# chensh236/ComputerVisionImageStich2

Measured on AMD Instinct MI355X. Metric: warp+blend MPix/s at 4096x4096x3 f32, higher is better.
Workload: dtype f32 (f64 accumulators)

## Files before the change

computervisionimagestich2_amd/csrc/k_sweeps.inc:

```
constexpr int TS = 64;
constexpr int TP = 68;

__device__ __forceinline__ void tile_load(const float* __restrict__ base, int pitch, int c0, int lane, f4 pre[16]) {
    const float* p = base + (size_t)(lane >> 4) * pitch + c0 + ((lane & 15) << 2);
#pragma unroll
    for (int i = 0; i < 16; ++i) pre[i] = *reinterpret_cast<const f4*>(p + (size_t)(4 * i) * pitch);
}
__device__ __forceinline__ void tile_to_lds(float* tile, int lane, const f4 pre[16]) {
    float* t = tile + (lane >> 4) * TP + ((lane & 15) << 2);
#pragma unroll
    for (int i = 0; i < 16; ++i) *reinterpret_cast<f4*>(t + (4 * i) * TP) = pre[i];
}
__device__ __forceinline__ void tile_store(float* __restrict__ base, int pitch, int c0, int lane, const float* tile) {
    float* p = base + (size_t)(lane >> 4) * pitch + c0 + ((lane & 15) << 2);
    const float* t = tile + (lane >> 4) * TP + ((lane & 15) << 2);
#pragma unroll
    for (int i = 0; i < 16; ++i)
        __builtin_nontemporal_store(*reinterpret_cast<const f4*>(t + (4 * i) * TP), reinterpret_cast<f4*>(p + (size_t)(4 * i) * pitch));
}

struct Bands {
    int nr, h;
};

struct MaskL0 {
    const SeamDev* seam;
    float* side;
    int h;
    int enabled;
};
__device__ __forceinline__ float mask_step(const SeamDev& sd, int x) {
    return sd.branch == 0 ? ((double)x < sd.thr ? 1.f : 0.f) : (x >= sd.start ? 1.f : 0.f);
}

__device__ __forceinline__ void tile_store_rows(float* __restrict__ base, int pitch, int c0, int lane, const float* tile, int nrows) {
    float* p = base + (size_t)(lane >> 4) * pitch + c0 + ((lane & 15) << 2);
    const float* t = tile + (lane >> 4) * TP + ((lane & 15) << 2);
#pragma unroll
    for (int i = 0; i < 16; ++i)
        if ((lane >> 4) + 4 * i < nrows)
            __builtin_nontemporal_store(*reinterpret_cast<const f4*>(t + (4 * i) * TP), reinterpret_cast<f4*>(p + (size_t)(4 * i) * pitch));
}

template <typename PX>
__device__ __forceinline__ void mosaic_indices(const XShift& ms, int c0, int lane, int y0, int w, f4 nidx[16]) {
    const int c = c0 + ((lane & 15) << 2);
    const unsigned c0i = mosaic_col<PX>(ms, c, w), c1i = mosaic_col<PX>(ms, c + 1, w), c2i = mosaic_col<PX>(ms, c + 2, w),
                   c3i = mosaic_col<PX>(ms, c + 3, w);
#pragma unroll
    for (int i = 0; i < 16; ++i) {
        const unsigned row = mosaic_row<PX>(ms, y0 + (lane >> 4) + 4 * i);
        f4 v;
        v.x = __uint_as_float(mosaic_offset<PX>(row, c0i));
        v.y = __uint_as_float(mosaic_offset<PX>(row, c1i));
        v.z = __uint_as_float(mosaic_offset<PX>(row, c2i));
        v.w = __uint_as_float(mosaic_offset<PX>(row, c3i));
        nidx[i] = v;
    }
}
template <typename PX>
__device__ __forceinline__ float src_px(__amdgpu_buffer_rsrc_t rs, bool warped, unsigned byte_off) {
    const float v = buf_px<PX>(rs, byte_off);
    return warped ? warped_px<PX>(v) : v;
}
template <typename PX>
__device__ __forceinline__ void src_gather(__amdgpu_buffer_rsrc_t rs, const f4 nidx[16], f4 pre[16]) {
#pragma unroll
    for (int i = 0; i < 16; ++i) {
        const f4 id = nidx[i];
        f4 v;
        v.x = buf_raw<PX>(rs, __float_as_uint(id.x));
        v.y = buf_raw<PX>(rs, __float_as_uint(id.y));
        v.z = buf_raw<PX>(rs, __float_as_uint(id.z));
        v.w = buf_raw<PX>(rs, __float_as_uint(id.w));
        pre[i] = v;
    }
}
template <typename PX>
__device__ __forceinline__ void src_finish(bool warped, f4 pre[16]) {
#pragma unroll
    for (int i = 0; i < 16; ++i) {
        f4 v = pre[i];
#pragma unroll
        for (int j = 0; j < 4; ++j) {
            const float t = raw_to_px<PX>(v[j]);
            v[j] = warped ? warped_px<PX>(t) : t;
        }
        pre[i] = v;
    }
}

template <typename PX, bool SRC, bool CKPT = false>
__global__ __launch_bounds__(64) void k_vv_x_fwd(const float* __restrict__ in, float* __restrict__ out, int w, int pitch,
                                                  long lines, VVK k, double* __restrict__ state, MaskL0 mk,
                                                  typename CollapseSrc<PX, SRC>::type pa, ZeroTiles zt, ZeroTiles zi,
                                                  double* __restrict__ ckpt, Bands bd) {
    __shared__ __attribute__((aligned(16))) float tile[TS * TP];
    const int lane = threadIdx.x;
    long blk = blockIdx.x;
    if (SRC && bd.nr > 0 && bd.nr % 8 == 0) {
        const long nr = bd.nr, per_pair = 7 * nr, pr_ = blk / per_pair, r = blk % per_pair;
        const long band = (r / 56) * 8 + r % 8, q = (r / 8) % 7;
        blk = pr_ * per_pair + q * nr + band;
    }
    const long plane = bd.nr > 0 ? blk / bd.nr : 0;
    const int band_y0 = bd.nr > 0 ? (int)(blk % bd.nr) * TS : 0;
    const int nrows = bd.nr > 0 ? min(TS, bd.h - band_y0) : TS;
    const long line0 = bd.nr > 0 ? plane * bd.h + band_y0 : blk * TS, line = line0 + lane;
    const float* ib = in + (size_t)line0 * pitch;
    float* ob = out + (size_t)line0 * pitch;
    const int ntiles = (w + TS - 1) / TS;
    const bool live = lane < nrows && line < lines;
    bool gen_mask = false;
    SeamDev sd;
    int src_q = 0, src_y0 = 0, src_pr = 0;
    if (mk.enabled) {
        if (plane % 7 == 6) {
            if (band_y0 >= TS) return;
            gen_mask = true;
            sd = mk.seam[plane / 7];
        }
        src_q = (int)(plane % 7);
        src_pr = (int)(plane / 7);
        src_y0 = band_y0;
    }
    const bool gen_frame = SRC && !gen_mask && src_q < 3 && !a_is_dense(pa), gen_mosaic = SRC && !gen_mask && !gen_frame;
    const __amdgpu_buffer_rsrc_t rs = x_rsrc<PX>(pa, src_pr, src_q);
    const XShift ms = x_shift<PX>(pa, src_pr, src_q);
    const float* idx_rows = in + ((size_t)src_pr * 7 * bd.h + src_y0) * pitch;
    f4 nidx[SRC ? 16 : 1];
    auto tile_outside = [&](int t) -> bool {
        if constexpr (SRC) return gen_frame && zi.flags && zi.flags[zi.index(src_pr, src_y0 >> 6, t)];
        return false;
    };
    auto index_tile = [&](int t) {
        if constexpr (SRC)
            if (!tile_outside(t)) tile_load(idx_rows, pitch, t * TS, lane, nidx);
    };
    auto gen_tile = [&](int c0, f4 pre[16]) {
        f4 v;
        const int c = c0 + ((lane & 15) << 2);
        v.x = mask_step(sd, c);
        v.y = mask_step(sd, c + 1);
        v.z = mask_step(sd, c + 2);
        v.w = mask_step(sd, c + 3);
#pragma unroll
        for (int i = 0; i < 16; ++i) pre[i] = v;
    };
    double iplus = 0.0;
    if (live)
        iplus = gen_mask     ? (double)mask_step(sd, w - 1)
                : gen_frame  ? (double)src_px<PX>(rs, true, reinterpret_cast<const unsigned*>(idx_rows)[(size_t)lane * pitch + (w - 1)])
                : gen_mosaic ? (double)src_px<PX>(rs, false, mosaic_offset<PX>(mosaic_row<PX>(ms, src_y0 + lane), mosaic_col<PX>(ms, w - 1, w)))
                             : (double)in[(size_t)line * pitch + (w - 1)];
    double v1 = 0, v2 = 0, v3 = 0;
    f4 pre[16];
#define STITCH_X_FETCH(T)                                                      \
    do {                                                                       \
        if (gen_mask)                                                          \
            gen_tile((T) * TS, pre);                                           \
        else if constexpr (SRC) {                                              \
            if (tile_outside(T)) {                                             \
                _Pragma("unroll") for (int i_ = 0; i_ < 16; ++i_) pre[i_] = f4{0.f, 0.f, 0.f, 0.f}; \
            } else                                                             \
                src_gather<PX>(rs, nidx, pre);                                 \
            if ((T) + 1 < ntiles) {                                            \
                if (gen_frame)                                                 \
                    index_tile((T) + 1);                                       \
                else                                                           \
                    mosaic_indices<PX>(ms, ((T) + 1) * TS, lane, src_y0, w, nidx); \
            }                                                                  \
        } else                                                                 \
            tile_load(ib, pitch, (T) * TS, lane, pre);                         \
    } while (0)
    if constexpr (SRC) {
        if (gen_frame)
            index_tile(0);
        else if (gen_mosaic)
            mosaic_indices<PX>(ms, 0, lane, src_y0, w, nidx);
    }
    STITCH_X_FETCH(0);
    for (int t = 0; t < ntiles; ++t) {
        if (!CKPT && zt.flags && tile_outside(t) &&
            (t == 0 || __ballot(live && (__double_as_longlong(v1) | __double_as_longlong(v2) | __double_as_longlong(v3)) != 0) == 0)) {
            if (t + 1 < ntiles) STITCH_X_FETCH(t + 1);
            if (lane == 0) zt.flags[zt.index(plane, band_y0 / TS, t)] = 1;
            continue;
        }
        if constexpr (SRC)
            if (!gen_mask) src_finish<PX>(gen_frame, pre);
        tile_to_lds(tile, lane, pre);
        if (t + 1 < ntiles) STITCH_X_FETCH(t + 1);
        __syncthreads();
        float* row = tile + lane * TP;
        const int jmax = min(TS, w - t * TS);
        if (t == 0) v1 = v2 = v3 = (double)row[0] / k.sumsq;
        if (CKPT && t > 0 && live) {
            double* c = ckpt + (size_t)(3 * t) * lines + line;
            c[0] = v1;
            c[lines] = v2;
            c[2 * lines] = v3;
        }
        const int jfull = jmax & ~15;
        unsigned nz = 0;
        for (int jb = 0; jb < jfull; jb += 16) {
            float xs[16];
#pragma unroll
            for (int q = 0; q < 4; ++q) *reinterpret_cast<f4*>(xs + 4 * q) = *reinterpret_cast<const f4*>(row + jb + 4 * q);
#pragma unroll
            for (int u = 0; u < 16; ++u) {
                double v0 = (double)xs[u];
                v0 += v1 * k.f1;
                v0 += v2 * k.f2;
                v0 += v3 * k.f3;
                xs[u] = (float)v0;
                nz |= __float_as_uint(xs[u]);
                v3 = v2;
                v2 = v1;
                v1 = v0;
            }
            if (!CKPT) {
#pragma unroll
                for (int q = 0; q < 4; ++q) *reinterpret_cast<f4*>(row + jb + 4 * q) = *reinterpret_cast<const f4*>(xs + 4 * q);
            }
        }
        for (int j = jfull; j < jmax; ++j) {
            double v0 = (double)row[j];
            v0 += v1 * k.f1;
            v0 += v2 * k.f2;
            v0 += v3 * k.f3;
            const float f = (float)v0;
            if (!CKPT) row[j] = f;
            nz |= __float_as_uint(f);
            v3 = v2;
            v2 = v1;
            v1 = v0;
        }
        __syncthreads();
        if (zt.flags) {
            const bool zero = __ballot(live && nz != 0) == 0;
            if (lane == 0) zt.flags[zt.index(plane, band_y0 / TS, t)] = zero ? 1 : 0;
            if (zero) continue;
        }
        if (!CKPT) {
            if (nrows == TS)
                tile_store(ob, pitch, t * TS, lane, tile);
            else
                tile_store_rows(ob, pitch, t * TS, lane, tile, nrows);
        }
    }
    if (live) {
        state[line] = v1;
        state[lines + line] = v2;
        state[2 * lines + line] = v3;
        state[3 * lines + line] = iplus;
    }
}

#undef STITCH_X_FETCH

__device__ __forceinline__ void triggs(const VVK& k, double iplus, double& v1, double& v2, double& v3, float& first) {
    const double uplus = iplus / k.den, vplus = uplus / k.den, unp = v1 - uplus, unp1 = v2 - uplus, unp2 = v3 - uplus;
    const double n0 = (k.M[0] * unp + k.M[1] * unp1 + k.M[2] * unp2 + vplus) * k.sum;
    const double n1 = (k.M[3] * unp + k.M[4] * unp1 + k.M[5] * unp2 + vplus) * k.sum;
    const double n2 = (k.M[6] * unp + k.M[7] * unp1 + k.M[8] * unp2 + vplus) * k.sum;
    first = (float)n0;
    v3 = n2;
    v2 = n1;
    v1 = n0;
}

__global__ __launch_bounds__(64) void k_vv_x_bwd(float* __restrict__ data, int w, int pitch, long lines, VVK k,
                                                  const double* __restrict__ state, MaskL0 mk, Bands bd) {
    __shared__ __attribute__((aligned(16))) float tile[TS * TP];
    const int lane = threadIdx.x;
    const long blk = blockIdx.x, plane = bd.nr > 0 ? blk / bd.nr : 0;
    const int band_y0 = bd.nr > 0 ? (int)(blk % bd.nr) * TS : 0;
    const int nrows = bd.nr > 0 ? min(TS, bd.h - band_y0) : TS;
    const long line0 = bd.nr > 0 ? plane * bd.h + band_y0 : blk * TS, line = line0 + lane;
    float* side_row = nullptr;
    if (mk.enabled) {
        if (plane % 7 == 6) {
            if (band_y0 >= TS) return;
            side_row = mk.side + (size_t)(plane / 7) * pitch;
        }
    }
    float* base = data + (size_t)line0 * pitch;
    const int ntiles = (w + TS - 1) / TS;
    const bool live = lane < nrows && line < lines;
    double v1 = 0, v2 = 0, v3 = 0, iplus = 0;
    if (live) {
        v1 = state[line];
        v2 = state[lines + line];
        v3 = state[2 * lines + line];
        iplus = state[3 * lines + line];
    }
    float first;
    triggs(k, iplus, v1, v2, v3, first);
    f4 pre[16];
    tile_load(base, pitch, (ntiles - 1) * TS, lane, pre);
    for (int t = ntiles - 1; t >= 0; --t) {
        tile_to_lds(tile, lane, pre);
        if (t > 0) tile_load(base, pitch, (t - 1) * TS, lane, pre);
        __syncthreads();
        float* row = tile + lane * TP;
        int jtop = min(TS, w - t * TS);
        if (t == ntiles - 1) {
            row[jtop - 1] = first;
            --jtop;
        }
        const int jfull = jtop & ~15;
        if (jtop > jfull) {
            for (int j = jtop - 1; j >= jfull; --j) {
                double v0 = (double)row[j];
                v0 *= k.sum;
                v0 += v1 * k.f1;
                v0 += v2 * k.f2;
                v0 += v3 * k.f3;
                row[j] = (float)v0;
                v3 = v2;
                v2 = v1;
                v1 = v0;
            }
        }
        for (int jb = jfull - 16; jb >= 0; jb -= 16) {
            float xs[16];
#pragma unroll
            for (int q = 0; q < 4; ++q) *reinterpret_cast<f4*>(xs + 4 * q) = *reinterpret_cast<const f4*>(row + jb + 4 * q);
#pragma unroll
            for (int u = 15; u >= 0; --u) {
                double v0 = (double)xs[u];
                v0 *= k.sum;
                v0 += v1 * k.f1;
                v0 += v2 * k.f2;
                v0 += v3 * k.f3;
                xs[u] = (float)v0;
                v3 = v2;
                v2 = v1;
// ... 462 lines not shown
```

computervisionimagestich2_amd/csrc/stitch_band.inc:

```
namespace {
constexpr int BAND_HALO = 2;

struct BandLevel {
    int w = 0, h_full = 0, rows = 0, row0 = 0, pitch = 0;
    int halo = 0;
    size_t ps = 0;
    float* g = nullptr;
    float* e = nullptr;
    int32_t *ix = nullptr, *iy = nullptr;
    double *ax = nullptr, *ay = nullptr;
    int c4_xa = 0, c4_xb = 0, sh_eff = 0;
    float* origin_g() const { return g + (size_t)halo * pitch; }
    float* origin_e() const { return e + (size_t)halo * pitch; }
};
}

struct stitch_band {
    int device = 0, cw = 0, ch = 0, rank = 0, nranks = 1, Ls = 0, L = 0;
    stitch_blend_opts opts{};
    VVK vvk{};
    BandLevel lv[32];
    void* arena = nullptr;
    size_t arena_bytes = 0;
    float* T = nullptr;
// ... 59 lines not shown
        const int ph = a.rows + 2 * a.halo, ybase = a.row0 - a.halo;
        PairArgs<PX>& px = band_pa<PX>(b, false);
        PairArgs<PX>& pc = band_pa<PX>(b, true);
        px = pa, pc = pa;
        px.oy[0] = oy + ybase, pc.oy[0] = oy + a.row0;
        const ZeroTiles zi = band_zero_tiles(b, b->zi);
        if (zi.flags) k_fill_bytes<<<64, 256, 0, s>>>(zi.flags, (size_t)zi.NR * zi.NC, (uint8_t)1);
        k_src_index<PX><<<grid_xy(a.pitch, (ph + SI_ROWS - 1) / SI_ROWS, 1), 256, 0, s>>>(pa, a.g, a.w, ph, a.pitch, a.ps, zi, ybase);
        k_seam<PX><<<1, 256, 0, s>>>(nullptr, b->cw, b->ch, a.pitch, a.ps, b->opts.seam_rule, b->d_seam, pa, 1);
    } else {
        k_compose<PX><<<grid_xy(a.pitch, a.rows, 1), 256, 0, s>>>(pa, a.origin_g(), a.w, a.rows, a.pitch, a.ps, a.row0);
        k_seam<PX><<<1, 256, 0, s>>>(nullptr, b->cw, b->ch, a.pitch, a.ps, b->opts.seam_rule, b->d_seam, pa, 1);
        k_mask<<<grid_xy(a.pitch, a.rows, 1), 256, 0, s>>>(a.origin_g(), a.w, a.pitch, a.ps, b->d_seam);
    }
    HIPCHK(hipMemcpyAsync(b->h_seam, b->d_seam, sizeof(SeamDev), hipMemcpyDeviceToHost, s));
    b->last_stream = s, b->pending = true;
    return launch_check("band_compose");
}

template <typename OUT>
int band_collapse(stitch_band* b, int level, OUT* d_out, void* stream) {
    int rc = band_check(b, level, b->Ls - 1);
    if (rc) return rc;
    if (level == 0 && !d_out) return fail(STITCH_ERR_ARG, "band_collapse: level 0 needs the output band");
    hipStream_t s = as_stream(stream);
    const BandLevel& a = b->lv[level];
    const BandLevel& nx = b->lv[level + 1];
    const bool top_src = level + 1 == b->Ls;
    const float* gn = top_src ? b->gtop : nx.g;
    const float* en = top_src ? b->etop : nx.e;
    const int spitch = top_src ? nx.w : nx.pitch;
    const size_t sps = top_src ? (size_t)nx.w * nx.h_full : nx.ps;
    int xa = a.c4_xa, xb = a.c4_xb;
    const int crows = std::max(4, std::min(32, a.rows / 8));
    const int strips = (a.rows + crows - 1) / crows;
    if (level == 0) {
        if ((a.w % 4) != 0 || (reinterpret_cast<uintptr_t>(d_out) % (4 * sizeof(OUT))) != 0) xa = xb = 0;
        OutPtrs<OUT> outs{};
        outs.p[0] = d_out;
        if (b->src_l0 && b->px != (int)sizeof(OUT)) return fail(STITCH_ERR_ARG, "band_collapse: the output's pixel type differs from the composed inputs'");
        CollapseArgs<OUT, true> A{a.origin_g(), a.w, a.rows, a.pitch, a.ps, gn, en, nx.w, a.sh_eff, spitch, sps, {a.ix, a.ax, a.iy, a.ay}, outs,
                                  a.w, (size_t)a.w * a.rows, b->d_seam, b->src_l0 ? band_pa<OUT>(b, true) : PairArgs<OUT>{}, b->src_l0 ? 1 : 0, crows, xa, xb,
                                  1};
        const int rest = a.w - (xb - xa), nb4 = ((xb - xa) / 4 + WAVE - 1) / WAVE, ncb = (rest + C4_THREADS - 1) / C4_THREADS;
        if (xb > xa)
            k_collapse4<OUT, true><<<dim3(nb4 + ncb * C4_SUB, strips, 1), C4_THREADS, 0, s>>>(A, nb4, ncb);
        else
            k_collapse<OUT, true><<<grid_xy(a.w, strips, 1), 256, 0, s>>>(A);
    } else {
        OutPtrs<float> eo{};
        eo.p[0] = a.origin_e();
        CollapseArgs<float, false> A{a.origin_g(), a.w, a.rows, a.pitch, a.ps, gn, en, nx.w, a.sh_eff, spitch, sps, {a.ix, a.ax, a.iy, a.ay}, eo,
                                     a.pitch, a.ps, nullptr, NoPairArgs{}, 0, crows, xa, xb, 1};
        const int rest = a.pitch - (xb - xa), nb4 = ((xb - xa) / 4 + WAVE - 1) / WAVE, ncb = (rest + C4_THREADS - 1) / C4_THREADS;
        if (xb > xa)
            k_collapse4<float, false><<<dim3(nb4 + ncb * C4_SUB, strips, 1), C4_THREADS, 0, s>>>(A, nb4, ncb);
        else
            k_collapse<float, false><<<grid_xy(a.pitch, strips, 1), 256, 0, s>>>(A);
    }
    b->last_stream = s, b->pending = true;
    return launch_check("band_collapse");
}
}

namespace {
Bands band_bands(const stitch_band* b) {
    const int ph = b->lv[0].rows + 2 * b->lv[0].halo;
    return Bands{(ph + TS - 1) / TS, ph};
}
ZeroTiles band_zero_tiles(const stitch_band* b, uint8_t* flags, int level) {
    const BandLevel& a = b->lv[level];
    ZeroTiles z{};
    const int NR = (a.rows + TS - 1) / TS;
    if ((level > 0 || b->src_l0) && (a.w & 1) == 0 && NR <= 256 && a.halo == 0 && b->zero_tiles && !b->plain_dec) {
        z.flags = flags;
        z.h = a.rows;
        z.NR = NR;
        z.NC = (a.w + TS - 1) / TS;
    }
    return z;
}
int band_x_fwd_src(stitch_band* b, hipStream_t s, bool flags) {
    const BandLevel& a = b->lv[0];
    const Bands bd = band_bands(b);
    const long lines = 7L * bd.h;
    const ZeroTiles zt = flags ? band_zero_tiles(b, b->zt) : ZeroTiles{}, zi = band_zero_tiles(b, b->zi);
    if (b->px == 1)
        k_vv_x_fwd<uint8_t, true><<<7 * bd.nr, 64, 0, s>>>(a.g, b->T, a.w, a.pitch, lines, b->vvk, b->state_x, band_mask(b), b->pa8x, zt, zi, nullptr, bd);
    else if (b->px == 4)
        k_vv_x_fwd<float, true><<<7 * bd.nr, 64, 0, s>>>(a.g, b->T, a.w, a.pitch, lines, b->vvk, b->state_x, band_mask(b), b->pafx, zt, zi, nullptr, bd);
    else
        return fail(STITCH_ERR_ARG, "band: reduce before compose");
    return STITCH_OK;
}
}

extern "C" {

int stitch_band_create(int cw, int ch, int rank, int nranks, int split_levels, const stitch_blend_opts* opts, stitch_band** out) {
    if (!out) return fail(STITCH_ERR_ARG, "band_create: null output");
    *out = nullptr;
    int rc = need_device();
    if (rc) return rc;
    stitch_blend_opts o;
    stitch_blend_opts_default(&o);
    if (opts) o = *opts;
    if (o.blur_kind != 0 || o.level_rule != 0 || o.seam_rule != 0 || !(o.sigma >= 0.5f))
        return fail(STITCH_ERR_ARG, "band_create: the band split implements the root variant (Van Vliet blur, sigma >= 0.5)");
    if (nranks < 1 || rank < 0 || rank >= nranks) return fail(STITCH_ERR_ARG, "band_create: rank %d of %d", rank, nranks);
    int lw[32], lh[32];
    const int L = pyramid_levels(cw, ch, 0, lw, lh);
    if (L < 0) return L;
    const int Ls = split_levels;
    if (Ls < 1 || Ls > L - 1) return fail(STITCH_ERR_ARG, "band_create: split_levels must be 1..%d for a %d-level pyramid", L - 1, L);
    for (int l = 0; l <= Ls; ++l) {
        const int q = l < Ls ? 2 * nranks : nranks;
        if (lh[l] % q != 0 || lh[l] / nranks < (l < Ls ? 2 * BAND_HALO : 1))
            return fail(STITCH_ERR_ARG, "band_create: level %d has %d rows, not divisible into %d bands of even height >= %d", l, lh[l], nranks,
                        2 * BAND_HALO);
        if (lw[l] < 2) return fail(STITCH_ERR_ARG, "band_create: level %d is %d columns wide", l, lw[l]);
    }
    stitch_band* b = new stitch_band();
    b->cw = cw, b->ch = ch, b->rank = rank, b->nranks = nranks, b->Ls = Ls, b->L = L, b->opts = o;
    b->vvk = make_vvk(o.sigma);
    if (hipGetDevice(&b->device) != hipSuccess) {
        delete b;
        return fail(STITCH_ERR_HIP, "hipGetDevice failed");
    }
    size_t off = 0;
    auto take = [&](size_t bytes) {
        const size_t o2 = off;
        off += align256(bytes);
        return o2;
    };
    size_t g_off[32], e_off[32], ix_off[32], ax_off[32], iy_off[32], ay_off[32];
    for (int l = 0; l <= Ls; ++l) {
        BandLevel& v = b->lv[l];
        v.w = lw[l], v.h_full = lh[l], v.rows = lh[l] / nranks, v.row0 = rank * v.rows, v.pitch = round_up(v.w, 64);
        v.halo = l == 0 || nranks == 1 ? 0 : BAND_HALO;
        v.ps = (size_t)v.pitch * (v.rows + 2 * v.halo);
        g_off[l] = take(sizeof(float) * (v.ps * 7 + (size_t)v.pitch * 64));
        e_off[l] = (l >= 1 && l < Ls) ? take(sizeof(float) * v.ps * 3) : 0;
        if (l < Ls) {
            ix_off[l] = take(sizeof(int32_t) * v.w);
            ax_off[l] = take(sizeof(double) * v.w);
            iy_off[l] = take(sizeof(int32_t) * v.rows);
            ay_off[l] = take(sizeof(double) * v.rows);
        }
    }
    const BandLevel& v0 = b->lv[0];
    const size_t t_off = take(sizeof(float) * (v0.ps * 7 + (size_t)v0.pitch * 64));
    const size_t st_off = take(sizeof(double) * 4 * 7 * (size_t)(v0.rows + 2 * BAND_HALO + 64));
    const size_t seam_off = take(sizeof(SeamDev));
    const size_t side_off = take(sizeof(float) * v0.pitch);
    const size_t ntile0 = (size_t)((v0.rows + TS - 1) / TS) * ((v0.w + TS - 1) / TS);
    const size_t zt_off = take(7 * ntile0), zi_off = take(ntile0);
    const size_t yg_off = take(sizeof(u64) * (7 * (size_t)(v0.pitch / TS) * WF_GRAN * WAVE + 1));
    const size_t wfc_off = take(sizeof(unsigned) * 64);
    const size_t gtop_off = take(sizeof(float) * 7 * (size_t)lw[Ls] * lh[Ls]);
    const size_t etop_off = take(sizeof(float) * 3 * (size_t)lw[Ls] * lh[Ls]);
    b->arena_bytes = off;
    if (hipMalloc(&b->arena, off) != hipSuccess || hipMemset(b->arena, 0, off) != hipSuccess ||
        hipHostMalloc((void**)&b->h_seam, sizeof(SeamDev)) != hipSuccess || hipHostMalloc((void**)&b->h_wf_sticky, sizeof(unsigned)) != hipSuccess) {
        (void)hipGetLastError();
        stitch_band_destroy(b);
        return fail(STITCH_ERR_HIP, "band_create: allocation of %zu bytes failed", off);
    }
    std::memset(b->h_seam, 0, sizeof(SeamDev));
    *b->h_wf_sticky = 0;
    char* base = static_cast<char*>(b->arena);
    b->mask_side = reinterpret_cast<float*>(base + side_off);
    b->zt = reinterpret_cast<uint8_t*>(base + zt_off);
    b->zi = reinterpret_cast<uint8_t*>(base + zi_off);
// ... 318 lines not shown
```

computervisionimagestich2_amd/csrc/stitch_hip.hip:

```cpp
#include <hip/hip_runtime.h>

#include <cmath>
#include <cstdarg>
#include <cstdio>
#include <cstdlib>
#include <algorithm>
#include <cstring>
#include <atomic>
#include <condition_variable>
#include <functional>
#include <list>
#include <mutex>
#include <string>
#include <thread>
#include <vector>

#include "stitch.h"
#include "stitch_kernels.hpp"

#pragma clang fp contract(off)

using namespace sk;

namespace {
// ... 288 lines not shown

struct StageTimer {
    stitch_plan* p;
    hipStream_t s;
    ProfRec r{};
    bool on;
    StageTimer(stitch_plan* plan, hipStream_t st, int stage, int level)
        : p(plan), s(st), on(plan->profiling && (plan->prof_only < 0 || plan->prof_only == stage)) {
        if (!on) return;
        r.stage = stage;
        r.level = level;
        auto get = [&](hipEvent_t& e) {
            if (!p->free_events.empty()) {
                e = p->free_events.back();
                p->free_events.pop_back();
            } else
                (void)hipEventCreate(&e);
        };
        get(r.a);
        get(r.b);
        (void)hipEventRecord(r.a, s);
    }
    ~StageTimer() {
        if (!on) return;
        (void)hipEventRecord(r.b, s);
        p->recs.push_back(r);
    }
};

dim3 grid_xy(int pitch_or_w, int h, int z = 1) { return dim3((pitch_or_w + 255) / 256, h, z); }

int launch_check(const char* what) {
    hipError_t e = hipGetLastError();
    if (e != hipSuccess) return fail(STITCH_ERR_HIP, "launch of %s failed: %s", what, hipGetErrorString(e));
    return STITCH_OK;
}

bool fused_sweep_call(const stitch_plan* p, int n) {
    return p->tune.wavefront >= 0 || p->tune.single_fast > 0 || n >= 2 || (p->tune.xbym == 0 && 7L * ((p->lv[0].h + TS - 1) / TS) >= 800);
}

bool lone_fused_level(const stitch_plan* p, int n, int l) {
    const Level& a = p->lv[l];
    const long mpix = p->tune.xbym > 0 ? 0 : p->tune.xbym_mpix >= 0 ? p->tune.xbym_mpix : 20;
    return n == 1 && p->wf_ctrl && l < 4 && p->opts.blur_kind == 0 && !p->blur_skip && p->tune.mover != 0 && p->tune.xbym != 0 && a.w > 1 && a.h > 1 &&
           (long)a.w * a.h >= mpix * 1000000L && (a.h + TS - 1) / TS < 4095 && !fused_sweep_call(p, n);
}

template <typename PX>
int run_reduce(stitch_plan* p, int n, hipStream_t s, const PairArgs<PX>& pa, bool src, const ZeroTiles& zi) {
    const int np = 7 * n;
    const bool any_lone_fused = lone_fused_level(p, n, 0);
    if (p->wf_levels > 0 || any_lone_fused) k_clear_words<<<1, 256, 0, s>>>((u64*)p->wf_ctrl, WF_CTRL_WORDS / 2);
    const int l_end = p->coarse_from > 0 ? p->coarse_from : p->L - 1;
    for (int l = 0; l < l_end; ++l) {
        const Level& a = p->lv[l];
        const Level& b = p->lv[l + 1];
        const long lines = (long)np * a.h;
        const bool do_x = a.w > 1 && !p->blur_skip, do_y = a.h > 1 && !p->blur_skip;
        bool decimated = false;
        MaskL0 mk{};
        if (l == 0 && p->mask_opt) {
            mk.seam = p->d_seam;
            mk.side = p->side;
            mk.h = a.h;
            mk.enabled = 1;
        }
        const bool wavefront = p->opts.blur_kind == 0 && do_x && do_y && l < p->wf_levels && fused_sweep_call(p, n);
        const bool odd_dec = (a.w & 1) != 0 && a.w >= 3 && !p->no_fuse && p->tune.odd_dec != 0;
        const int NR = (a.h + TS - 1) / TS;
        ZeroTiles zt{};
        const int nbx_bands = np * NR;
        const bool xby_zt = !wavefront && p->zt && do_x && do_y && lone_fused_level(p, n, l) && (a.w + TS - 1) / TS <= XY_MAXNC &&
                            !(p->tune.mover != 0 && (nbx_bands <= 340 || (src && l == 0 && nbx_bands <= 1024)));
        if ((wavefront || xby_zt) && p->zero_tiles && NR <= 256 && ((a.w & 1) == 0 || odd_dec) && !p->no_fuse && !(p->tune.gate64 && (a.h % TS || (a.w & 1)))) {
            zt.flags = p->zt;
            zt.h = a.h;
            zt.NR = NR;
            zt.NC = (a.w + TS - 1) / TS;
        }
        Bands bd{};
        if (mk.enabled || (src && l == 0) || zt.flags) bd = Bands{NR, a.h};
        const int nbx = bd.nr ? np * bd.nr : (int)((lines + TS - 1) / TS);
        const bool rowz = zt.flags && (a.h % YCH) != 0;
        if (wavefront) {
            const int nb = nbx;
            const bool rcmp = (p->recompute == 1 || (p->recompute == 2 && l >= 1)) && !(p->wf_dbg && l == 0);
            {
                StageTimer t(p, s, src && l == 0 ? STITCH_K_VV_X_FWD_SRC : STITCH_K_VV_X_FWD, l);
                if (src && l == 0) {
                    if (rcmp)
                        k_vv_x_fwd<PX, true, true><<<nb, 64, 0, s>>>(a.g, p->T, a.w, a.pitch, lines, p->vvk, p->state, mk, pa, zt, zi, p->ckpt, bd);
                    else
                        k_vv_x_fwd<PX, true><<<nb, 64, 0, s>>>(a.g, p->T, a.w, a.pitch, lines, p->vvk, p->state, mk, pa, zt, zi, nullptr, bd);
                } else if (rcmp)
                    k_vv_x_fwd<PX, false, true><<<nb, 64, 0, s>>>(a.g, p->T, a.w, a.pitch, lines, p->vvk, p->state, mk, NoPairArgs{}, zt, ZeroTiles{}, p->ckpt, bd);
                else
                    k_vv_x_fwd<PX, false><<<nb, 64, 0, s>>>(a.g, p->T, a.w, a.pitch, lines, p->vvk, p->state, mk, NoPairArgs{}, zt, ZeroTiles{}, nullptr, bd);
            }
            Wavefront wf{};
            wf.yg = p->wf_yg;
            wf.counter = p->wf_ctrl + (size_t)l * 16;
            wf.abort = p->wf_ctrl + WF_CTRL_WORDS - 16;
            wf.sticky = p->wf_ctrl + WF_CTRL_WORDS;
            wf.spin_limit = p->wf_spin_limit;
            wf.NR = NR;
            wf.NC = (a.w + TS - 1) / TS;
            wf.NP = np;
            const size_t gran_words = (size_t)wf.NP * wf.NC * WF_GRAN * WAVE;
            k_clear_words<<<(int)std::min<size_t>((gran_words + 255) / 256, 2048), 256, 0, s>>>(p->wf_yg, gran_words);
            wf.epoch = 1;
            wf.mask_l0 = mk.enabled;
            wf.zt = zt;
            wf.early_read = p->wf_early_read;
            const long ntiles = (long)wf.NP * wf.NR;
            double* state_y = p->state + 4 * (size_t)p->cap * 7 * (a.h + 64);
            {
                StageTimer t(p, s, STITCH_K_VV_XBYF, l);
                const int wg = (int)std::min<long>(ntiles, p->wf_max_wgs);
                Recompute rcv{};
                if (rcmp) {
                    rcv.in = a.g;
                    rcv.ckpt = p->ckpt;
                    rcv.seam = p->d_seam;
                    if (src && l == 0) rcv.zi = zi;
                }
                if (p->wf_dbg && l == 0) {
                    wf.dbg = p->wf_dbg;
                    k_vv_xbyf<true><<<wg, 64, 0, s>>>(p->T, a.w, a.h, a.pitch, p->vvk, p->state, lines, state_y, wf, rcv, NoPairArgs{});
                } else if (rcmp && src && l == 0)
                    k_vv_xbyf<false, PX, 2><<<wg, 64, 0, s>>>(p->T, a.w, a.h, a.pitch, p->vvk, p->state, lines, state_y, wf, rcv, pa);
                else if (rcmp)
                    k_vv_xbyf<false, float, 1><<<wg, 64, 0, s>>>(p->T, a.w, a.h, a.pitch, p->vvk, p->state, lines, state_y, wf, rcv, NoPairArgs{});
                else
                    k_vv_xbyf<false><<<wg, 64, 0, s>>>(p->T, a.w, a.h, a.pitch, p->vvk, p->state, lines, state_y, wf, rcv, NoPairArgs{});
            }
            StageTimer t(p, s, STITCH_K_VV_Y_BWD, l);
            dim3 g((a.pitch + YCOLS - 1) / YCOLS, np);
            if ((a.w & 1) == 0 && !p->no_fuse) {
                if (rowz)
                    k_vv_y_bwd_dec<true><<<g, 128, 0, s>>>(p->T, a.w, a.h, a.pitch, a.ps, p->vvk, state_y, b.g, b.w, b.h, b.pitch, b.ps, zt, nullptr, nullptr, a.h, b.h);
                else
                    k_vv_y_bwd_dec<false><<<g, 128, 0, s>>>(p->T, a.w, a.h, a.pitch, a.ps, p->vvk, state_y, b.g, b.w, b.h, b.pitch, b.ps, zt, nullptr, nullptr, a.h, b.h);
                decimated = true;
            } else if (odd_dec) {
                const dim3 go((b.w + WAVE - 2) / (WAVE - 1), np);
                if (rowz)
                    k_vv_y_bwd_dec<true, YST, true, true><<<go, 128, 0, s>>>(p->T, a.w, a.h, a.pitch, a.ps, p->vvk, state_y, b.g, b.w, b.h, b.pitch, b.ps, zt, nullptr, nullptr, a.h, b.h);
                else
                    k_vv_y_bwd_dec<false, YST, true, true><<<go, 128, 0, s>>>(p->T, a.w, a.h, a.pitch, a.ps, p->vvk, state_y, b.g, b.w, b.h, b.pitch, b.ps, zt, nullptr, nullptr, a.h, b.h);
                decimated = true;
            } else
                k_vv_y_bwd<<<g, 64, 0, s>>>(p->T, a.h, a.pitch, a.ps, p->vvk, state_y, nullptr, nullptr);
        } else if (p->opts.blur_kind == 0) {
            const bool mover = p->tune.mover != 0;
            const bool src0 = src && l == 0;
            const bool xby = do_x && do_y && lone_fused_level(p, n, l);
            const double* ystate = p->state;
            if (do_x && mover && !zt.flags && (nbx <= 340 || (src0 && nbx <= 1024))) {
                {
                    StageTimer t(p, s, src0 ? STITCH_K_VV_X_FWD_SRC : STITCH_K_VV_X_FWD, l);
                    if (src0)
                        k_vv_x_m<true, PX, true><<<nbx, 192, 0, s>>>(a.g, p->T, a.w, a.pitch, lines, p->vvk, p->state, mk, bd, pa);
                    else
                        k_vv_x_m<true><<<nbx, 192, 0, s>>>(a.g, p->T, a.w, a.pitch, lines, p->vvk, p->state, mk, bd, NoPairArgs{});
                }
                StageTimer t(p, s, STITCH_K_VV_X_BWD, l);
                if (xby) {
                } else if (nbx <= 340)
                    k_vv_x_m<false><<<nbx, 192, 0, s>>>(p->T, p->T, a.w, a.pitch, lines, p->vvk, p->state, mk, bd, NoPairArgs{});
                else
                    k_vv_x_bwd<<<nbx, 64, 0, s>>>(p->T, a.w, a.pitch, lines, p->vvk, p->state, mk, bd);
            } else if (do_x) {
                const int nb = nbx;
                {
                    StageTimer t(p, s, src && l == 0 ? STITCH_K_VV_X_FWD_SRC : STITCH_K_VV_X_FWD, l);
                    if (src && l == 0)
                        k_vv_x_fwd<PX, true><<<nb, 64, 0, s>>>(a.g, p->T, a.w, a.pitch, lines, p->vvk, p->state, mk, pa, zt, zi, nullptr, bd);
                    else
                        k_vv_x_fwd<PX, false><<<nb, 64, 0, s>>>(a.g, p->T, a.w, a.pitch, lines, p->vvk, p->state, mk, NoPairArgs{}, zt, ZeroTiles{}, nullptr, bd);
                }
                if (!xby) {
                    StageTimer t(p, s, STITCH_K_VV_X_BWD, l);
                    k_vv_x_bwd<<<nb, 64, 0, s>>>(p->T, a.w, a.pitch, lines, p->vvk, p->state, mk, bd);
                }
            } else
                HIPCHK(hipMemcpyAsync(p->T, a.g, sizeof(float) * a.ps * np, hipMemcpyDeviceToDevice, s));
            if (xby) {
                Wavefront wf{};
                wf.yg = p->wf_yg;
                wf.counter = p->wf_ctrl + (size_t)l * 16;
                wf.abort = p->wf_ctrl + WF_CTRL_WORDS - 16;
                wf.sticky = p->wf_ctrl + WF_CTRL_WORDS;
                wf.spin_limit = p->wf_spin_limit;
                wf.NR = NR;
                wf.NC = (a.w + TS - 1) / TS;
                wf.NP = np;
                wf.epoch = 1;
                wf.mask_l0 = mk.enabled;
                wf.zt = zt;
                if (p->xy_dbg && l == 0) wf.dbg = p->xy_dbg, p->xy_dbg_nc = wf.NC;
                const size_t gran_words = (size_t)wf.NP * wf.NC * WF_GRAN * WAVE;
                k_clear_words<<<(int)std::min<size_t>((gran_words + 255) / 256, 2048), 256, 0, s>>>(p->wf_yg, gran_words);
                double* state_y = p->state + 4 * (size_t)p->cap * 7 * (a.h + 64);
                ystate = state_y;
                StageTimer t(p, s, STITCH_K_VV_XBYF, l);
                k_vv_xby_m<<<(int)std::min<long>((long)wf.NP * wf.NR, XY_WGS), XY_THREADS, 0, s>>>(p->T, a.w, a.h, a.pitch, p->vvk, p->state, lines, state_y, wf, p->zero_page);
            }
            if (do_y) {
                dim3 g((a.pitch + YCOLS - 1) / YCOLS, np);
                const bool lone = (long)g.x * g.y < 1536 && !p->tune.y2, small_plane = a.ps * sizeof(float) < 0x7fffffffULL;
                const bool ymover = mover && lone && (long)(a.pitch / WAVE) * np <= 340;
                if (!xby) {
                    StageTimer t(p, s, STITCH_K_VV_Y_FWD, l);
                    if (ymover)
                        k_vv_y_m<true><<<dim3(a.pitch / WAVE, np), 192, 0, s>>>(p->T, a.h, a.pitch, a.ps, p->vvk, p->state, mk);
                    else if (lone && small_plane && p->tune.y1s != 0 && (p->tune.y1s >= 2 || a.ps * np * sizeof(float) * 2 < (1000u << 20)))
                        k_vv_y_fwd1s<8><<<dim3(a.pitch / WAVE, np), 64, 0, s>>>(p->T, a.h, a.pitch, a.ps, p->vvk, p->state, mk, nullptr);
                    else if (lone)
                        k_vv_y_fwd1<<<dim3(a.pitch / WAVE, np), 64, 0, s>>>(p->T, a.h, a.pitch, a.ps, p->vvk, p->state, mk, nullptr);
                    else
                        k_vv_y_fwd<<<g, 64, 0, s>>>(p->T, a.h, a.pitch, a.ps, p->vvk, p->state, mk, nullptr);
                }
                StageTimer t(p, s, STITCH_K_VV_Y_BWD, l);
                const bool dec7 = lone && small_plane && p->tune.dec7 != 0 && !zt.flags;
                if (zt.flags && ((a.w & 1) == 0 || odd_dec) && !p->no_fuse) {
                    if ((a.w & 1) == 0) {
                        if (rowz)
                            k_vv_y_bwd_dec<true><<<g, 128, 0, s>>>(p->T, a.w, a.h, a.pitch, a.ps, p->vvk, ystate, b.g, b.w, b.h, b.pitch, b.ps, zt, nullptr, nullptr, a.h, b.h);
                        else
                            k_vv_y_bwd_dec<false><<<g, 128, 0, s>>>(p->T, a.w, a.h, a.pitch, a.ps, p->vvk, ystate, b.g, b.w, b.h, b.pitch, b.ps, zt, nullptr, nullptr, a.h, b.h);
                    } else {
                        const dim3 go((b.w + WAVE - 2) / (WAVE - 1), np);
                        if (rowz)
                            k_vv_y_bwd_dec<true, YST, true, true><<<go, 128, 0, s>>>(p->T, a.w, a.h, a.pitch, a.ps, p->vvk, ystate, b.g, b.w, b.h, b.pitch, b.ps, zt, nullptr, nullptr, a.h, b.h);
                        else
                            k_vv_y_bwd_dec<false, YST, true, true><<<go, 128, 0, s>>>(p->T, a.w, a.h, a.pitch, a.ps, p->vvk, ystate, b.g, b.w, b.h, b.pitch, b.ps, zt, nullptr, nullptr, a.h, b.h);
                    }
                    decimated = true;
                } else if ((a.w & 1) == 0 && !p->no_fuse) {
                    if (dec7) {
                        unsigned long long* dbg = p->d7_dbg && l == p->d7_dbg_level ? p->d7_dbg : nullptr;
                        if (dbg) p->d7_dbg_chunks = (a.h + YCH - 1) / YCH;
                        k_vv_y_bwd_dec7<false><<<g, D7_THREADS, 0, s>>>(p->T, a.w, a.h, a.pitch, a.ps, p->vvk, ystate, b.g, b.w, b.h, b.pitch, b.ps, dbg, dbg ? Tuning::env_int("STITCH_D7_STAMP_MODE") : 0);
                    }
                    else
                        k_vv_y_bwd_dec<false, YST, false><<<g, 128, 0, s>>>(p->T, a.w, a.h, a.pitch, a.ps, p->vvk, ystate, b.g, b.w, b.h, b.pitch, b.ps, ZeroTiles{}, nullptr, nullptr, a.h, b.h);
                    decimated = true;
                } else if (odd_dec) {
                    const dim3 go((b.w + WAVE - 2) / (WAVE - 1), np);
                    if (dec7)
                        k_vv_y_bwd_dec7<true><<<go, D7_THREADS, 0, s>>>(p->T, a.w, a.h, a.pitch, a.ps, p->vvk, ystate, b.g, b.w, b.h, b.pitch, b.ps);
                    else
                        k_vv_y_bwd_dec<false, YST, false, true><<<go, 128, 0, s>>>(p->T, a.w, a.h, a.pitch, a.ps, p->vvk, ystate, b.g, b.w, b.h, b.pitch, b.ps, ZeroTiles{}, nullptr, nullptr, a.h, b.h);
                    decimated = true;
                } else
                    k_vv_y_bwd<<<g, 64, 0, s>>>(p->T, a.h, a.pitch, a.ps, p->vvk, ystate, nullptr, nullptr);
            }
        } else {
            HIPCHK(hipMemcpyAsync(p->T, a.g, sizeof(float) * a.ps * np, hipMemcpyDeviceToDevice, s));
            if (do_x) {
// ... 1787 lines not shown
```

Before: 24540.

## Process three warped color channels per block in source x-forward sweep

In the source x-forward recursive-filter pass, each block now handles the three frame channels together, so the gather index tile is loaded once and reused for all three channels. It also adds a remapped block grid, a direct b128 buffer load for shift-only mosaic tiles that sit fully inside the source, and skipping of mosaic tiles outside the source. The filter state becomes per-channel arrays and occupancy is hinted with launch_bounds(64,2). Costs include more registers, less parallelism for the frame planes, and moving the iplus state write to an earlier point.

```diff
diff --git a/computervisionimagestich2_amd/csrc/k_sweeps.inc b/computervisionimagestich2_amd/csrc/k_sweeps.inc
--- a/computervisionimagestich2_amd/csrc/k_sweeps.inc
+++ b/computervisionimagestich2_amd/csrc/k_sweeps.inc
@@ -19,9 +19,18 @@
         __builtin_nontemporal_store(*reinterpret_cast<const f4*>(t + (4 * i) * TP), reinterpret_cast<f4*>(p + (size_t)(4 * i) * pitch));
 }
 
+#ifndef STITCH_XSRC_TRIPLE
+#define STITCH_XSRC_TRIPLE 1
+#endif
+#ifndef STITCH_XSRC_WIDE
+#define STITCH_XSRC_WIDE 1
+#endif
+
 struct Bands {
     int nr, h;
+    int triple;
 };
+inline int src_triple_blocks(int n, int nr) { return n * (4 * nr + 1); }
 
 struct MaskL0 {
     const SeamDev* seam;
@@ -77,6 +86,15 @@
     }
 }
 template <typename PX>
+__device__ __forceinline__ void shift_tile_load(__amdgpu_buffer_rsrc_t rs, const XShift& ms, int c0, int lane, int y0, f4 pre[16]) {
+    if constexpr (sizeof(PX) == 4) {
+        const unsigned pitch_b = (unsigned)ms.mw * 4u;
+        const unsigned o = (unsigned)(y0 + ms.oy + (lane >> 4)) * pitch_b + (unsigned)(c0 + ms.ox + ((lane & 15) << 2)) * 4u;
+#pragma unroll
+        for (int i = 0; i < 16; ++i) pre[i] = __builtin_bit_cast(f4, __builtin_amdgcn_raw_buffer_load_b128(rs, o + (unsigned)(4 * i) * pitch_b, 0, 0));
+    }
+}
+template <typename PX>
 __device__ __forceinline__ void src_finish(bool warped, f4 pre[16]) {
 #pragma unroll
     for (int i = 0; i < 16; ++i) {
@@ -91,14 +109,25 @@
 }
 
 template <typename PX, bool SRC, bool CKPT = false>
-__global__ __launch_bounds__(64) void k_vv_x_fwd(const float* __restrict__ in, float* __restrict__ out, int w, int pitch,
+__global__ __launch_bounds__(64, 2) void k_vv_x_fwd(const float* __restrict__ in, float* __restrict__ out, int w, int pitch,
                                                   long lines, VVK k, double* __restrict__ state, MaskL0 mk,
                                                   typename CollapseSrc<PX, SRC>::type pa, ZeroTiles zt, ZeroTiles zi,
                                                   double* __restrict__ ckpt, Bands bd) {
+    constexpr int NCH = SRC && !CKPT ? 3 : 1;
     __shared__ __attribute__((aligned(16))) float tile[TS * TP];
     const int lane = threadIdx.x;
     long blk = blockIdx.x;
-    if (SRC && bd.nr > 0 && bd.nr % 8 == 0) {
+    if (NCH == 3 && bd.triple) {
+        const long nr = bd.nr, nf = lines / (7L * bd.h) * nr;
+        long pr_, q, band = blk % nr;
+        if (blk < nf)
+            pr_ = blk / nr, q = 0;
+        else if (blk < 4 * nf)
+            pr_ = (blk - nf) / (3 * nr), q = 3 + (blk - nf) / nr % 3;
+        else
+            pr_ = blk - 4 * nf, q = 6, band = 0;
+        blk = (pr_ * 7 + q) * nr + band;
+    } else if (SRC && bd.nr > 0 && bd.nr % 8 == 0) {
         const long nr = bd.nr, per_pair = 7 * nr, pr_ = blk / per_pair, r = blk % per_pair;
         const long band = (r / 56) * 8 + r % 8, q = (r / 8) % 7;
         blk = pr_ * per_pair + q * nr + band;
@@ -125,12 +154,26 @@
         src_y0 = band_y0;
     }
     const bool gen_frame = SRC && !gen_mask && src_q < 3 && !a_is_dense(pa), gen_mosaic = SRC && !gen_mask && !gen_frame;
-    const __amdgpu_buffer_rsrc_t rs = x_rsrc<PX>(pa, src_pr, src_q);
+    const int nch = NCH == 3 && bd.triple && gen_frame ? 3 : 1;
+    __amdgpu_buffer_rsrc_t rs[NCH];
+#pragma unroll
+    for (int c = 0; c < NCH; ++c) rs[c] = x_rsrc<PX>(pa, src_pr, src_q + c);
     const XShift ms = x_shift<PX>(pa, src_pr, src_q);
     const float* idx_rows = in + ((size_t)src_pr * 7 * bd.h + src_y0) * pitch;
     f4 nidx[SRC ? 16 : 1];
+    auto shift_class = [&](int t) -> int {
+        const long long x0 = (long long)t * TS + ms.ox, y0 = (long long)src_y0 + ms.oy;
+        if (x0 + TS <= 0 || x0 >= ms.mw || y0 + nrows <= 0 || y0 >= ms.mh) return 0;
+#if STITCH_XSRC_WIDE
+        if (sizeof(PX) == 4 && t * TS + TS <= w && x0 >= 0 && x0 + TS <= ms.mw && y0 >= 0 && y0 + TS <= ms.mh) return 2;
+#endif
+        return 1;
+    };
     auto tile_outside = [&](int t) -> bool {
-        if constexpr (SRC) return gen_frame && zi.flags && zi.flags[zi.index(src_pr, src_y0 >> 6, t)];
+        if constexpr (SRC) {
+            if (gen_frame) return zi.flags && zi.flags[zi.index(src_pr, src_y0 >> 6, t)];
+            return STITCH_XSRC_WIDE && gen_mosaic && shift_class(t) == 0;
+        }
         return false;
     };
     auto index_tile = [&](int t) {
@@ -147,113 +190,132 @@
 #pragma unroll
         for (int i = 0; i < 16; ++i) pre[i] = v;
     };
-    double iplus = 0.0;
-    if (live)
-        iplus = gen_mask     ? (double)mask_step(sd, w - 1)
-                : gen_frame  ? (double)src_px<PX>(rs, true, reinterpret_cast<const unsigned*>(idx_rows)[(size_t)lane * pitch + (w - 1)])
-                : gen_mosaic ? (double)src_px<PX>(rs, false, mosaic_offset<PX>(mosaic_row<PX>(ms, src_y0 + lane), mosaic_col<PX>(ms, w - 1, w)))
-                             : (double)in[(size_t)line * pitch + (w - 1)];
-    double v1 = 0, v2 = 0, v3 = 0;
+    double v1[NCH], v2[NCH], v3[NCH];
+#pragma unroll
+    for (int c = 0; c < NCH; ++c) v1[c] = v2[c] = v3[c] = 0.0;
+    if (live) {
+        double* ip = state + 3 * lines + line;
+        if (gen_frame) {
+            const unsigned io = reinterpret_cast<const unsigned*>(idx_rows)[(size_t)lane * pitch + (w - 1)];
+#pragma unroll
+            for (int c = 0; c < NCH; ++c)
+                if (c < nch) ip[(long)c * bd.h] = (double)src_px<PX>(rs[c], true, io);
+        } else
+            ip[0] = gen_mask     ? (double)mask_step(sd, w - 1)
+                    : gen_mosaic ? (double)src_px<PX>(rs[0], false, mosaic_offset<PX>(mosaic_row<PX>(ms, src_y0 + lane), mosaic_col<PX>(ms, w - 1, w)))
+                                 : (double)in[(size_t)line * pitch + (w - 1)];
+    }
     f4 pre[16];
-#define STITCH_X_FETCH(T)                                                      \
+#define STITCH_X_FETCH(T, RS, LAST)                                            \
     do {                                                                       \
         if (gen_mask)                                                          \
             gen_tile((T) * TS, pre);                                           \
         else if constexpr (SRC) {                                              \
             if (tile_outside(T)) {                                             \
                 _Pragma("unroll") for (int i_ = 0; i_ < 16; ++i_) pre[i_] = f4{0.f, 0.f, 0.f, 0.f}; \
-            } else                                                             \
-                src_gather<PX>(rs, nidx, pre);                                 \
-            if ((T) + 1 < ntiles) {                                            \
-                if (gen_frame)                                                 \
-                    index_tile((T) + 1);                                       \
-                else                                                           \
-                    mosaic_indices<PX>(ms, ((T) + 1) * TS, lane, src_y0, w, nidx); \
+            } else if (gen_mosaic && shift_class(T) == 2)                      \
+                shift_tile_load<PX>(RS, ms, (T) * TS, lane, src_y0, pre); \
+            else {                                                             \
+                if (gen_mosaic) mosaic_indices<PX>(ms, (T) * TS, lane, src_y0, w, nidx); \
+                src_gather<PX>(RS, nidx, pre);                                 \
             }                                                                  \
+            if (gen_frame && (LAST) && (T) + 1 < ntiles) index_tile((T) + 1);  \
         } else                                                                 \
             tile_load(ib, pitch, (T) * TS, lane, pre);                         \
     } while (0)
-    if constexpr (SRC) {
-        if (gen_frame)
-            index_tile(0);
-        else if (gen_mosaic)
-            mosaic_indices<PX>(ms, 0, lane, src_y0, w, nidx);
-    }
-    STITCH_X_FETCH(0);
+    if constexpr (SRC)
+        if (gen_frame) index_tile(0);
+    STITCH_X_FETCH(0, rs[0], nch == 1);
     for (int t = 0; t < ntiles; ++t) {
-        if (!CKPT && zt.flags && tile_outside(t) &&
-            (t == 0 || __ballot(live && (__double_as_longlong(v1) | __double_as_longlong(v2) | __double_as_longlong(v3)) != 0) == 0)) {
-            if (t + 1 < ntiles) STITCH_X_FETCH(t + 1);
-            if (lane == 0) zt.flags[zt.index(plane, band_y0 / TS, t)] = 1;
-            continue;
-        }
-        if constexpr (SRC)
-            if (!gen_mask) src_finish<PX>(gen_frame, pre);
-        tile_to_lds(tile, lane, pre);
-        if (t + 1 < ntiles) STITCH_X_FETCH(t + 1);
-        __syncthreads();
-        float* row = tile + lane * TP;
-        const int jmax = min(TS, w - t * TS);
-        if (t == 0) v1 = v2 = v3 = (double)row[0] / k.sumsq;
-        if (CKPT && t > 0 && live) {
-            double* c = ckpt + (size_t)(3 * t) * lines + line;
-            c[0] = v1;
-            c[lines] = v2;
-            c[2 * lines] = v3;
-        }
-        const int jfull = jmax & ~15;
-        unsigned nz = 0;
-        for (int jb = 0; jb < jfull; jb += 16) {
-            float xs[16];
-#pragma unroll
-            for (int q = 0; q < 4; ++q) *reinterpret_cast<f4*>(xs + 4 * q) = *reinterpret_cast<const f4*>(row + jb + 4 * q);
-#pragma unroll
-            for (int u = 0; u < 16; ++u) {
-                double v0 = (double)xs[u];
-                v0 += v1 * k.f1;
-                v0 += v2 * k.f2;
-                v0 += v3 * k.f3;
-                xs[u] = (float)v0;
-                nz |= __float_as_uint(xs[u]);
-                v3 = v2;
-                v2 = v1;
-                v1 = v0;
+#pragma unroll
+        for (int c = 0; c < NCH; ++c) {
+            if (c >= nch) break;
+            const long cline = line + (long)c * bd.h;
+            float* cob = ob + (size_t)c * bd.h * pitch;
+            const bool skip = !CKPT && zt.flags && tile_outside(t) &&
+                              (t == 0 || __ballot(live && (__double_as_longlong(v1[c]) | __double_as_longlong(v2[c]) | __double_as_longlong(v3[c])) != 0) == 0);
+            if (!skip) {
+                if constexpr (SRC)
+                    if (!gen_mask) src_finish<PX>(gen_frame, pre);
+                tile_to_lds(tile, lane, pre);
+            }
+            {
+                const bool wrap = c + 1 == nch;
+                const int nt = wrap ? t + 1 : t, cn = c + 1 < NCH ? c + 1 : 0;
+                if (nt < ntiles) STITCH_X_FETCH(nt, wrap ? rs[0] : rs[cn], wrap ? nch == 1 : cn + 1 == nch);
+            }
+            if (skip) {
+                if (lane == 0) zt.flags[zt.index(plane + c, band_y0 / TS, t)] = 1;
+                continue;
+            }
+            __syncthreads();
+            float* row = tile + lane * TP;
+            const int jmax = min(TS, w - t * TS);
+            if (t == 0) v1[c] = v2[c] = v3[c] = (double)row[0] / k.sumsq;
+            if (CKPT && t > 0 && live) {
+                double* cp = ckpt + (size_t)(3 * t) * lines + cline;
+                cp[0] = v1[c];
+                cp[lines] = v2[c];
+                cp[2 * lines] = v3[c];
+            }
+            const int jfull = jmax & ~15;
+            unsigned nz = 0;
+            for (int jb = 0; jb < jfull; jb += 16) {
+                float xs[16];
+#pragma unroll
+                for (int q = 0; q < 4; ++q) *reinterpret_cast<f4*>(xs + 4 * q) = *reinterpret_cast<const f4*>(row + jb + 4 * q);
+#pragma unroll
+                for (int u = 0; u < 16; ++u) {
+                    double v0 = (double)xs[u];
+                    v0 += v1[c] * k.f1;
+                    v0 += v2[c] * k.f2;
+                    v0 += v3[c] * k.f3;
+                    xs[u] = (float)v0;
+                    nz |= __float_as_uint(xs[u]);
+                    v3[c] = v2[c];
+                    v2[c] = v1[c];
+                    v1[c] = v0;
+                }
+                if (!CKPT) {
+#pragma unroll
+                    for (int q = 0; q < 4; ++q) *reinterpret_cast<f4*>(row + jb + 4 * q) = *reinterpret_cast<const f4*>(xs + 4 * q);
+                }
+            }
+            for (int j = jfull; j < jmax; ++j) {
+                double v0 = (double)row[j];
+                v0 += v1[c] * k.f1;
+                v0 += v2[c] * k.f2;
+                v0 += v3[c] * k.f3;
+                const float f = (float)v0;
+                if (!CKPT) row[j] = f;
+                nz |= __float_as_uint(f);
+                v3[c] = v2[c];
+                v2[c] = v1[c];
+                v1[c] = v0;
+            }
+            __syncthreads();
+            if (zt.flags) {
+                const bool zero = __ballot(live && nz != 0) == 0;
+                if (lane == 0) zt.flags[zt.index(plane + c, band_y0 / TS, t)] = zero ? 1 : 0;
+                if (zero) continue;
             }
             if (!CKPT) {
-#pragma unroll
-                for (int q = 0; q < 4; ++q) *reinterpret_cast<f4*>(row + jb + 4 * q) = *reinterpret_cast<const f4*>(xs + 4 * q);
-            }
-        }
-        for (int j = jfull; j < jmax; ++j) {
-            double v0 = (double)row[j];
-            v0 += v1 * k.f1;
-            v0 += v2 * k.f2;
-            v0 += v3 * k.f3;
-            const float f = (float)v0;
-            if (!CKPT) row[j] = f;
-            nz |= __float_as_uint(f);
-            v3 = v2;
-            v2 = v1;
-            v1 = v0;
-        }
-        __syncthreads();
-        if (zt.flags) {
-            const bool zero = __ballot(live && nz != 0) == 0;
-            if (lane == 0) zt.flags[zt.index(plane, band_y0 / TS, t)] = zero ? 1 : 0;
-            if (zero) continue;
-        }
-        if (!CKPT) {
-            if (nrows == TS)
-                tile_store(ob, pitch, t * TS, lane, tile);
-            else
-                tile_store_rows(ob, pitch, t * TS, lane, tile, nrows);
+                if (nrows == TS)
+                    tile_store(cob, pitch, t * TS, lane, tile);
+                else
+                    tile_store_rows(cob, pitch, t * TS, lane, tile, nrows);
+            }
         }
     }
     if (live) {
-        state[line] = v1;
-        state[lines + line] = v2;
-        state[2 * lines + line] = v3;
-        state[3 * lines + line] = iplus;
+#pragma unroll
+        for (int c = 0; c < NCH; ++c)
+            if (c < nch) {
+                const long cline = line + (long)c * bd.h;
+                state[cline] = v1[c];
+                state[lines + cline] = v2[c];
+                state[2 * lines + cline] = v3[c];
+            }
     }
 }
 
diff --git a/computervisionimagestich2_amd/csrc/stitch_band.inc b/computervisionimagestich2_amd/csrc/stitch_band.inc
--- a/computervisionimagestich2_amd/csrc/stitch_band.inc
+++ b/computervisionimagestich2_amd/csrc/stitch_band.inc
@@ -165,13 +165,15 @@
 }
 int band_x_fwd_src(stitch_band* b, hipStream_t s, bool flags) {
     const BandLevel& a = b->lv[0];
-    const Bands bd = band_bands(b);
+    Bands bd = band_bands(b);
+    bd.triple = STITCH_XSRC_TRIPLE;
+    const int nb = bd.triple ? src_triple_blocks(1, bd.nr) : 7 * bd.nr;
     const long lines = 7L * bd.h;
     const ZeroTiles zt = flags ? band_zero_tiles(b, b->zt) : ZeroTiles{}, zi = band_zero_tiles(b, b->zi);
     if (b->px == 1)
-        k_vv_x_fwd<uint8_t, true><<<7 * bd.nr, 64, 0, s>>>(a.g, b->T, a.w, a.pitch, lines, b->vvk, b->state_x, band_mask(b), b->pa8x, zt, zi, nullptr, bd);
+        k_vv_x_fwd<uint8_t, true><<<nb, 64, 0, s>>>(a.g, b->T, a.w, a.pitch, lines, b->vvk, b->state_x, band_mask(b), b->pa8x, zt, zi, nullptr, bd);
     else if (b->px == 4)
-        k_vv_x_fwd<float, true><<<7 * bd.nr, 64, 0, s>>>(a.g, b->T, a.w, a.pitch, lines, b->vvk, b->state_x, band_mask(b), b->pafx, zt, zi, nullptr, bd);
+        k_vv_x_fwd<float, true><<<nb, 64, 0, s>>>(a.g, b->T, a.w, a.pitch, lines, b->vvk, b->state_x, band_mask(b), b->pafx, zt, zi, nullptr, bd);
     else
         return fail(STITCH_ERR_ARG, "band: reduce before compose");
     return STITCH_OK;
diff --git a/computervisionimagestich2_amd/csrc/stitch_hip.hip b/computervisionimagestich2_amd/csrc/stitch_hip.hip
--- a/computervisionimagestich2_amd/csrc/stitch_hip.hip
+++ b/computervisionimagestich2_amd/csrc/stitch_hip.hip
@@ -394,6 +394,9 @@
         Bands bd{};
         if (mk.enabled || (src && l == 0) || zt.flags) bd = Bands{NR, a.h};
         const int nbx = bd.nr ? np * bd.nr : (int)((lines + TS - 1) / TS);
+        Bands src_bd = bd;
+        src_bd.triple = STITCH_XSRC_TRIPLE && src && l == 0 && mk.enabled && !pa.a_dense;
+        const int src_nb = src_bd.triple ? src_triple_blocks(n, bd.nr) : nbx;
         const bool rowz = zt.flags && (a.h % YCH) != 0;
         if (wavefront) {
             const int nb = nbx;
@@ -404,7 +407,7 @@
                     if (rcmp)
                         k_vv_x_fwd<PX, true, true><<<nb, 64, 0, s>>>(a.g, p->T, a.w, a.pitch, lines, p->vvk, p->state, mk, pa, zt, zi, p->ckpt, bd);
                     else
-                        k_vv_x_fwd<PX, true><<<nb, 64, 0, s>>>(a.g, p->T, a.w, a.pitch, lines, p->vvk, p->state, mk, pa, zt, zi, nullptr, bd);
+                        k_vv_x_fwd<PX, true><<<src_nb, 64, 0, s>>>(a.g, p->T, a.w, a.pitch, lines, p->vvk, p->state, mk, pa, zt, zi, nullptr, src_bd);
                 } else if (rcmp)
                     k_vv_x_fwd<PX, false, true><<<nb, 64, 0, s>>>(a.g, p->T, a.w, a.pitch, lines, p->vvk, p->state, mk, NoPairArgs{}, zt, ZeroTiles{}, p->ckpt, bd);
                 else
@@ -488,7 +491,7 @@
                 {
                     StageTimer t(p, s, src && l == 0 ? STITCH_K_VV_X_FWD_SRC : STITCH_K_VV_X_FWD, l);
                     if (src && l == 0)
-                        k_vv_x_fwd<PX, true><<<nb, 64, 0, s>>>(a.g, p->T, a.w, a.pitch, lines, p->vvk, p->state, mk, pa, zt, zi, nullptr, bd);
+                        k_vv_x_fwd<PX, true><<<src_nb, 64, 0, s>>>(a.g, p->T, a.w, a.pitch, lines, p->vvk, p->state, mk, pa, zt, zi, nullptr, src_bd);
                     else
                         k_vv_x_fwd<PX, false><<<nb, 64, 0, s>>>(a.g, p->T, a.w, a.pitch, lines, p->vvk, p->state, mk, NoPairArgs{}, zt, ZeroTiles{}, nullptr, bd);
                 }
```

Result: no change. 24340 (-0.8%).
